# stephanieleroux/sitrack

Measured on AMD Instinct MI355X. Metric: particle-steps/s, higher is better.
Workload: dtype f64

## Files before the change

include/sitrk.h:

```cpp
#ifndef SITRK_H
#define SITRK_H

#include <stdint.h>

#ifdef __cplusplus
extern "C" {
#endif

#define SITRK_VERSION 100

#define SITRK_OK        0
#define SITRK_EINVAL  (-1)
#define SITRK_EINDEX  (-2)
#define SITRK_EHIP    (-3)
#define SITRK_ENOMEM  (-4)

#define SITRK_F32 0
#define SITRK_F64 1

#define SITRK_FILL (-9999.0)

typedef struct sitrk_ctx sitrk_t;

int         sitrk_version(void);
// ... 1 lines not shown
int         sitrk_destroy(sitrk_t *h);
const char *sitrk_last_error(sitrk_t *h);
int         sitrk_sync(sitrk_t *h);
int         sitrk_set_stream(sitrk_t *h, void *hip_stream);

int sitrk_set_grid(sitrk_t *h, int Nj, int Ni,
                   const double *Yf, const double *Xf,
                   const double *Yu, const double *Xu,
                   const double *Yv, const double *Xv,
                   const int8_t *tmask);

int sitrk_set_params(sitrk_t *h, double rdt, int uv_strategy, double rmin_conc);

int sitrk_set_substeps(sitrk_t *h, int nsub);

int sitrk_set_tuning(sitrk_t *h, const char *knob, int value);

int   sitrk_alloc_records(sitrk_t *h, int nslots, int dtype);
int   sitrk_push_record(sitrk_t *h, int slot, const void *u, const void *v, const void *sic);
int   sitrk_stage_acquire(sitrk_t *h, int nrows, void **u, void **v, void **sic);
int   sitrk_stage_submit(sitrk_t *h, int slot, int j0, int j1);
int   sitrk_stage_release(sitrk_t *h);
int   sitrk_push_record_dev(sitrk_t *h, int slot, const void *slab_dev);
void *sitrk_record_ptr(sitrk_t *h, int slot);
int   sitrk_commit_record(sitrk_t *h, int slot);

int sitrk_buoy_rows(sitrk_t *h, int32_t *jmin, int32_t *jmax);
int sitrk_push_record_rows(sitrk_t *h, int slot, int j0, int j1, const void *u_rows, const void *v_rows, const void *sic_rows);
int sitrk_commit_record_rows(sitrk_t *h, int slot, int j0, int j1);

int sitrk_buoy_box(sitrk_t *h, int32_t *jmin, int32_t *jmax, int32_t *imin, int32_t *imax);
int sitrk_push_record_box(sitrk_t *h, int slot, int j0, int j1, int i0, int i1, const void *u_box, const void *v_box, const void *sic_box,
                          int64_t ld);
int sitrk_buoy_box_begin(sitrk_t *h);
int sitrk_buoy_box_end(sitrk_t *h, int32_t *jmin, int32_t *jmax, int32_t *imin, int32_t *imax, int32_t *age);
int sitrk_stage_acquire_box(sitrk_t *h, int nrows, int ncols, void **u, void **v, void **sic);
int sitrk_stage_submit_box(sitrk_t *h, int slot, int j0, int j1, int i0, int i1);
int sitrk_commit_record_box(sitrk_t *h, int slot, int j0, int j1, int i0, int i1);
int sitrk_commit_records_box(sitrk_t *h, int slot0, int nrec, int j0, int j1, int i0, int i1);
int sitrk_commit_records_box_async(sitrk_t *h, int slot0, int nrec, int j0, int j1, int i0, int i1);

int sitrk_set_buoys(sitrk_t *h, int64_t nP, const double *yx, const int32_t *jiT,
                    const int32_t *rec_first, const int32_t *rec_last);

int sitrk_restore_state(sitrk_t *h, const int8_t *alive, const int32_t *kill_rec);

int sitrk_sort_buoys(sitrk_t *h);
int sitrk_set_resort(sitrk_t *h, int resort_every);

int sitrk_step(sitrk_t *h, int slot, int jrec);

int sitrk_run(sitrk_t *h, int slot0, int jrec0, int nsteps);
int sitrk_launch_stats(sitrk_t *h, int reset, int64_t *fused_launches, int64_t *fused_records, int64_t *step_launches);

int sitrk_fetch(sitrk_t *h, double *yx, int32_t *jiT, int8_t *alive, int32_t *kill_rec);

int sitrk_fetch_record(sitrk_t *h, int jrec, double *yx_rec, int8_t *mask, double *latlon);

int sitrk_find_cells(sitrk_t *h, int64_t n, const double *yx, const int32_t *jiT_guess,
                     int32_t *jiT_out, int8_t *found);

int sitrk_seed_init(sitrk_t *h, int64_t nP, const double *latlon, const double *yx,
                    const double *latT, const double *lonT, const double *resolkm,
                    const double *sic, int32_t *jiT_out, int8_t *keep, int8_t *why);

int sitrk_nearest_point(sitrk_t *h, int64_t nP, const double *latlon, const double *latT, const double *lonT,
                        const double *resolkm, double rd_found_km, int max_itr, int32_t *ji, double *dmin);

int sitrk_nemo_seed(sitrk_t *h, int Nj, int Ni, int khss, const int8_t *tmask, const int8_t *rmask,
                    const double *latT, const double *lonT, const double *sic, const double *latF, const double *lonF,
                    double lat0, double lon0, int64_t capacity, double *latlon, double *yx, int64_t *nT, int64_t *nF);

int sitrk_subsample_cloud(sitrk_t *h, int64_t n, const double *yx, double rd_km, int8_t *keep, int64_t *nkeep, int32_t *launches);

int sitrk_cancel_too_close(sitrk_t *h, int64_t n, const double *lat, const double *lon, const int8_t *valid, const int32_t *nrec_all,
                           const int32_t *nrec_before, double rd_km, int8_t *keep, int64_t *nkeep, int64_t *nclose);

int sitrk_nearest_buoy(sitrk_t *h, int64_t n, const double *lat, const double *lon, const int8_t *valid, double rd_km, int32_t *nn,
                       double *dmin);

int sitrk_eval_inside(sitrk_t *h, int64_t n, const double *pts, const double *quads, int8_t *inside);
int sitrk_eval_euler(sitrk_t *h, int64_t n, const double *r, const double *vel, double rdt, double *out);
int sitrk_eval_haversine(sitrk_t *h, int64_t n, const double *plat, const double *plon, const double *xlat,
                         const double *xlon, double *dist);
int sitrk_eval_intersect(sitrk_t *h, int64_t n, const double *segs, int8_t *intersect, int8_t *ccw_abc);
int sitrk_eval_crossing(sitrk_t *h, int64_t n, const double *P1, const double *P2, const int32_t *jiT, int32_t *jiT_new,
                        int32_t *codes);
int sitrk_survive_mask(sitrk_t *h, const double *sic, int8_t *mask);

int sitrk_cart2geo(sitrk_t *h, int64_t n, const double *yx, double lat0, double lon0, double *latlon);
int sitrk_geo2cart(sitrk_t *h, int64_t n, const double *latlon, double lat0, double lon0, double *yx);

int sitrk_timer_start(sitrk_t *h);
int sitrk_timer_stop(sitrk_t *h, float *ms);
int sitrk_count_alive(sitrk_t *h, int64_t *nalive);

#ifdef __cplusplus
}
#endif
#endif
```

sitrack_amd/_lib.py:

```python
import ctypes as C
import os
import subprocess

import numpy as np

_HERE = os.path.dirname(os.path.abspath(__file__))
SO_PATH = os.environ.get("SITRK_LIB_PATH") or os.path.join(_HERE, "libsitrk.so")
CSRC = os.path.join(_HERE, "csrc")

SITRK_F32, SITRK_F64 = 0, 1
FillValue = -9999.0

_vp = C.c_void_p
_i64 = C.c_int64
_int = C.c_int
_dbl = C.c_double

_SIGNATURES = {
    "sitrk_version": (_int, []),
    "sitrk_create": (_int, [C.POINTER(_vp), _int]),
    "sitrk_destroy": (_int, [_vp]),
    "sitrk_last_error": (C.c_char_p, [_vp]),
    "sitrk_sync": (_int, [_vp]),
    "sitrk_set_stream": (_int, [_vp, _vp]),
    "sitrk_set_grid": (_int, [_vp, _int, _int] + [_vp] * 7),
    "sitrk_set_params": (_int, [_vp, _dbl, _int, _dbl]),
    "sitrk_set_substeps": (_int, [_vp, _int]),
    "sitrk_set_tuning": (_int, [_vp, C.c_char_p, _int]),
    "sitrk_alloc_records": (_int, [_vp, _int, _int]),
    "sitrk_push_record": (_int, [_vp, _int, _vp, _vp, _vp]),
    "sitrk_push_record_dev": (_int, [_vp, _int, _vp]),
    "sitrk_stage_acquire": (_int, [_vp, _int, C.POINTER(_vp), C.POINTER(_vp), C.POINTER(_vp)]),
    "sitrk_stage_submit": (_int, [_vp, _int, _int, _int]),
    "sitrk_stage_release": (_int, [_vp]),
    "sitrk_launch_stats": (_int, [_vp, _int, C.POINTER(_i64), C.POINTER(_i64), C.POINTER(_i64)]),
    "sitrk_buoy_rows": (_int, [_vp, C.POINTER(C.c_int32), C.POINTER(C.c_int32)]),
    "sitrk_push_record_rows": (_int, [_vp, _int, _int, _int, _vp, _vp, _vp]),
    "sitrk_commit_record_rows": (_int, [_vp, _int, _int, _int]),
    "sitrk_buoy_box": (_int, [_vp] + [C.POINTER(C.c_int32)] * 4),
    "sitrk_push_record_box": (_int, [_vp, _int, _int, _int, _int, _int, _vp, _vp, _vp, _i64]),
    "sitrk_buoy_box_begin": (_int, [_vp]),
    "sitrk_buoy_box_end": (_int, [_vp] + [C.POINTER(C.c_int32)] * 5),
    "sitrk_stage_acquire_box": (_int, [_vp, _int, _int, C.POINTER(_vp), C.POINTER(_vp), C.POINTER(_vp)]),
    "sitrk_stage_submit_box": (_int, [_vp, _int, _int, _int, _int, _int]),
    "sitrk_commit_record_box": (_int, [_vp, _int, _int, _int, _int, _int]),
    "sitrk_commit_records_box": (_int, [_vp, _int, _int, _int, _int, _int, _int]),
    "sitrk_commit_records_box_async": (_int, [_vp, _int, _int, _int, _int, _int, _int]),
    "sitrk_record_ptr": (_vp, [_vp, _int]),
    "sitrk_commit_record": (_int, [_vp, _int]),
    "sitrk_set_buoys": (_int, [_vp, _i64, _vp, _vp, _vp, _vp]),
    "sitrk_restore_state": (_int, [_vp, _vp, _vp]),
    "sitrk_sort_buoys": (_int, [_vp]),
    "sitrk_set_resort": (_int, [_vp, _int]),
    "sitrk_step": (_int, [_vp, _int, _int]),
    "sitrk_run": (_int, [_vp, _int, _int, _int]),
    "sitrk_fetch": (_int, [_vp, _vp, _vp, _vp, _vp]),
    "sitrk_fetch_record": (_int, [_vp, _int, _vp, _vp, _vp]),
    "sitrk_count_alive": (_int, [_vp, C.POINTER(_i64)]),
    "sitrk_find_cells": (_int, [_vp, _i64, _vp, _vp, _vp, _vp]),
    "sitrk_seed_init": (_int, [_vp, _i64] + [_vp] * 9),
    "sitrk_nemo_seed": (_int, [_vp, _int, _int, _int] + [_vp] * 7 + [_dbl, _dbl, _i64, _vp, _vp, C.POINTER(_i64), C.POINTER(_i64)]),
    "sitrk_subsample_cloud": (_int, [_vp, _i64, _vp, _dbl, _vp, C.POINTER(_i64), C.POINTER(C.c_int32)]),
    "sitrk_cancel_too_close": (_int, [_vp, _i64, _vp, _vp, _vp, _vp, _vp, _dbl, _vp, C.POINTER(_i64), C.POINTER(_i64)]),
    "sitrk_nearest_buoy": (_int, [_vp, _i64, _vp, _vp, _vp, _dbl, _vp, _vp]),
    "sitrk_nearest_point": (_int, [_vp, _i64, _vp, _vp, _vp, _vp, _dbl, _int, _vp, _vp]),
    "sitrk_eval_haversine": (_int, [_vp, _i64, _vp, _vp, _vp, _vp, _vp]),
    "sitrk_eval_inside": (_int, [_vp, _i64, _vp, _vp, _vp]),
    "sitrk_eval_euler": (_int, [_vp, _i64, _vp, _vp, _dbl, _vp]),
    "sitrk_eval_intersect": (_int, [_vp, _i64, _vp, _vp, _vp]),
    "sitrk_eval_crossing": (_int, [_vp, _i64, _vp, _vp, _vp, _vp, _vp]),
    "sitrk_survive_mask": (_int, [_vp, _vp, _vp]),
    "sitrk_cart2geo": (_int, [_vp, _i64, _vp, _dbl, _dbl, _vp]),
    "sitrk_geo2cart": (_int, [_vp, _i64, _vp, _dbl, _dbl, _vp]),
    "sitrk_timer_start": (_int, [_vp]),
    "sitrk_timer_stop": (_int, [_vp, C.POINTER(C.c_float)]),
}


class SitrkError(RuntimeError):
    pass


def build(force=False, verbose=False):
    cmd = ["make", "-C", CSRC] + (["-B"] if force else [])
    r = subprocess.run(cmd, capture_output=True, text=True)
    if verbose or r.returncode:
        print(r.stdout + r.stderr)
    if r.returncode:
# ... 131 lines not shown
            raise ValueError("records must be float32 or float64")
        self._chk(self._L.sitrk_alloc_records(self._h, int(nslots), SITRK_F64 if dt == np.float64 else SITRK_F32))
        self.nslots = int(nslots)
        self.field_dtype = dt

    def push_record(self, slot, u, v, sic):
        shp = (self.Nj, self.Ni)
        u = as_c(u, self.field_dtype, shp, "u")
        v = as_c(v, self.field_dtype, shp, "v")
        sic = as_c(sic, self.field_dtype, shp, "sic")
        self._chk(self._L.sitrk_push_record(self._h, int(slot), _ptr(u), _ptr(v), _ptr(sic)))

    def stage(self, nrows=None, ncols=None):
        nrows = self.Nj if nrows is None else int(nrows)
        ncols = self.Ni if ncols is None else int(ncols)
        pu, pv, ps = _vp(), _vp(), _vp()
        if ncols == self.Ni:
            self._chk(self._L.sitrk_stage_acquire(self._h, nrows, C.byref(pu), C.byref(pv), C.byref(ps)))
        else:
            self._chk(self._L.sitrk_stage_acquire_box(self._h, nrows, ncols, C.byref(pu), C.byref(pv), C.byref(ps)))
        nb = nrows * ncols * self.field_dtype.itemsize

        def view(p):
            return np.frombuffer((C.c_char * nb).from_address(p.value), dtype=self.field_dtype).reshape(nrows, ncols)
        self._staged_rows, self._staged_cols = nrows, ncols
        return view(pu), view(pv), view(ps)

    def stage_release(self):
        self._chk(self._L.sitrk_stage_release(self._h))

    def stage_fill(self, slot, j0, nrows, fill, i0=0, ncols=None):
        bufs = self.stage(nrows, ncols)
        try:
            fill(*bufs)
        except BaseException:
            self.stage_release()
            raise
        finally:
            del bufs
        self.submit(slot, j0, i0)

    def submit(self, slot, j0=0, i0=0):
        j1, i1 = int(j0) + int(self._staged_rows), int(i0) + int(self._staged_cols)
        if int(i0) == 0 and i1 == self.Ni:
            self._chk(self._L.sitrk_stage_submit(self._h, int(slot), int(j0), j1))
        else:
            self._chk(self._L.sitrk_stage_submit_box(self._h, int(slot), int(j0), j1, int(i0), i1))

    def launch_stats(self, reset=False):
        a, b, c = _i64(0), _i64(0), _i64(0)
        self._chk(self._L.sitrk_launch_stats(self._h, int(bool(reset)), C.byref(a), C.byref(b), C.byref(c)))
        return {"fused_launches": a.value, "fused_records": b.value, "step_launches": c.value}

    def buoy_rows(self):
        a, b = C.c_int32(0), C.c_int32(0)
        self._chk(self._L.sitrk_buoy_rows(self._h, C.byref(a), C.byref(b)))
        return a.value, b.value

    def band(self, age=0):
        jmin, jmax = self.buoy_rows()
        if jmin > jmax:
            return 0, 0
        d = reach(age, self.nsub)
        return max(0, jmin - 2 - d), min(self.Nj, jmax + 3 + d)

    def buoy_box(self):
        v = [C.c_int32(0) for _ in range(4)]
        self._chk(self._L.sitrk_buoy_box(self._h, *[C.byref(x) for x in v]))
        return tuple(x.value for x in v)

    def box(self, age=0, align=4):
        jmin, jmax, imin, imax = self.buoy_box()
        return self.box_of(jmin, jmax, imin, imax, age, align)

    def box_of(self, jmin, jmax, imin, imax, age=0, align=4):
        if jmin > jmax:
            return 0, 0, 0, 0
        d = reach(age, getattr(self, "nsub", 1))
        i0, i1 = max(0, imin - 2 - d), min(self.Ni, imax + 3 + d)
        i0 -= i0 % align
        i1 = min(self.Ni, -(-i1 // align) * align)
        return max(0, jmin - 2 - d), min(self.Nj, jmax + 3 + d), i0, i1

    def push_record_box(self, slot, j0, j1, i0, i1, u_box, v_box, sic_box):
        shp = (j1 - j0, i1 - i0)
        es = self.field_dtype.itemsize
        arrs = [np.asarray(x) for x in (u_box, v_box, sic_box)]
        for x, n in zip(arrs, ("u box", "v box", "sic box")):
            if tuple(x.shape) != shp:
                raise ValueError("%s: expected shape %s, got %s" % (n, shp, tuple(x.shape)))
        pitched = all(x.dtype == self.field_dtype and x.ndim == 2 and x.strides[1] == es and x.strides[0] % es == 0
                      and x.strides[0] >= shp[1] * es for x in arrs) and len({x.strides[0] for x in arrs}) == 1
        if pitched and shp[0] > 0 and shp[1] > 0:
            ld = arrs[0].strides[0] // es
        else:
            arrs = [as_c(x, self.field_dtype, shp) for x in arrs]
            ld = shp[1]
        self._chk(self._L.sitrk_push_record_box(self._h, int(slot), int(j0), int(j1), int(i0), int(i1), *[_ptr(x) for x in arrs], int(ld)))

    def buoy_box_begin(self):
        self._chk(self._L.sitrk_buoy_box_begin(self._h))

    def buoy_box_end(self):
        v = [C.c_int32(0) for _ in range(5)]
        self._chk(self._L.sitrk_buoy_box_end(self._h, *[C.byref(x) for x in v]))
        return tuple(x.value for x in v)
# ... 259 lines not shown
```

sitrack_amd/csrc/sitrk.hip:

```cpp
#include <hip/hip_runtime.h>

#include <algorithm>
#include <cmath>
#include <cstdarg>
#include <cstdio>
#include <cstring>
#include <new>
#include <thread>
#include <vector>

#include "../../include/sitrk.h"
#include "sitrk_internal.h"
#include "sitrk_kernels.h"
#include "sitrk_locate.h"
#include "sitrk_seed.h"

using namespace sitrk;

#define SITRK_API extern "C" __attribute__((visibility("default")))

static thread_local char g_create_err[512] = {0};

static int fail(sitrk_ctx *h, int code, const char *fmt, ...)
{
// ... 36 lines not shown
    dev_free(h->scratch);
    h->scratch = nullptr;
    h->scratch_bytes = 0;
    HIPCHK(hipMalloc(&h->scratch, bytes));
    h->scratch_bytes = bytes;
    return SITRK_OK;
}

static void free_buoys(sitrk_ctx *h)
{
    for (int b = 0; b < 2; b++) {
        dev_free(h->st[b].pos); dev_free(h->st[b].cell); dev_free(h->st[b].kill_rec);
        dev_free(h->st[b].win); dev_free(h->st[b].perm);
        h->st[b] = BuoyState();
        dev_free(h->keys[b]); dev_free(h->vals[b]);
        h->keys[b] = nullptr; h->vals[b] = nullptr;
    }
    dev_free(h->sort_tmp);
    h->sort_tmp = nullptr; h->sort_tmp_bytes = 0;
    h->nP = 0;
}

static void free_records(sitrk_ctx *h);

SITRK_API int sitrk_version(void) { return SITRK_VERSION; }

SITRK_API const char *sitrk_last_error(sitrk_t *h) { return h ? h->err : g_create_err; }

SITRK_API int sitrk_create(sitrk_t **out, int device)
{
    sitrk_ctx *h = nullptr;
    if (!out) return fail(h, SITRK_EINVAL, "sitrk_create: null output pointer");
    *out = nullptr;
    int ndev = 0;
    hipError_t e = hipGetDeviceCount(&ndev);
    if (e != hipSuccess || ndev <= 0)
        return fail(h, SITRK_EHIP, "sitrk_create: no HIP device (%s); libsitrk has no CPU path",
                    e == hipSuccess ? "device count 0" : hipGetErrorString(e));
    if (device < 0 || device >= ndev) return fail(h, SITRK_EINVAL, "sitrk_create: device %d out of range [0,%d)", device, ndev);
    e = hipSetDevice(device);
    if (e != hipSuccess) return fail(h, SITRK_EHIP, "hipSetDevice(%d) -> %s", device, hipGetErrorString(e));
    sitrk_ctx *c = new (std::nothrow) sitrk_ctx();
    if (!c) return fail(h, SITRK_ENOMEM, "sitrk_create: out of host memory");
    c->device = device;
    for (int k = 0; k < 4096; k++) c->slot_used_seq[k] = -1;
    e = hipStreamCreateWithFlags(&c->own_stream, hipStreamNonBlocking);
    if (e == hipSuccess) e = hipStreamCreateWithFlags(&c->copy_stream, hipStreamNonBlocking);
    if (e == hipSuccess) e = hipStreamCreateWithFlags(&c->sv_stream, hipStreamNonBlocking);
    if (e == hipSuccess) e = hipEventCreate(&c->ev0);
    if (e == hipSuccess) e = hipEventCreate(&c->ev1);
    for (int b = 0; b < sitrk_ctx::kStage && e == hipSuccess; b++) e = hipEventCreateWithFlags(&c->stage_done[b], hipEventDisableTiming);
    for (int k = 0; k < sitrk_ctx::kLaunchRing && e == hipSuccess; k++) e = hipEventCreateWithFlags(&c->launch_ev[k], hipEventDisableTiming);
    if (e == hipSuccess) e = hipEventCreateWithFlags(&c->box_ev, hipEventDisableTiming);
    if (e == hipSuccess) e = hipHostMalloc((void **)&c->box_host, 4 * sizeof(int), hipHostMallocDefault);
    if (e == hipSuccess) e = hipMalloc((void **)&c->counter, 4 * sizeof(unsigned long long));
    if (e != hipSuccess) {
        int rc = fail(h, SITRK_EHIP, "sitrk_create: %s", hipGetErrorString(e));
        (void)sitrk_destroy(c);
        return rc;
    }
    c->stream = c->own_stream;
    *out = c;
    return SITRK_OK;
}

SITRK_API int sitrk_destroy(sitrk_t *h)
{
    if (!h) return SITRK_OK;
    (void)hipSetDevice(h->device);
    if (h->copy_stream) (void)hipStreamSynchronize(h->copy_stream);
    if (h->sv_stream) (void)hipStreamSynchronize(h->sv_stream);
    if (h->stream) (void)hipStreamSynchronize(h->stream);
    free_buoys(h);
    free_records(h);
    dev_free(h->geo); dev_free(h->geoF); dev_free(h->orient); dev_free(h->tmask); dev_free(h->scratch); dev_free(h->counter);
    if (h->box_ev) (void)hipEventDestroy(h->box_ev);
    if (h->box_host) (void)hipHostFree(h->box_host);
    if (h->ev0) (void)hipEventDestroy(h->ev0);
    if (h->ev1) (void)hipEventDestroy(h->ev1);
    for (int b = 0; b < sitrk_ctx::kStage; b++) if (h->stage_done[b]) (void)hipEventDestroy(h->stage_done[b]);
    for (int k = 0; k < sitrk_ctx::kLaunchRing; k++) if (h->launch_ev[k]) (void)hipEventDestroy(h->launch_ev[k]);
    for (int k = 0; k < 4096; k++) if (h->slot_ready[k]) (void)hipEventDestroy(h->slot_ready[k]);
    for (int k = 0; k < 4096; k++) if (h->slot_sv[k]) (void)hipEventDestroy(h->slot_sv[k]);
    if (h->sv_stream) (void)hipStreamDestroy(h->sv_stream);
    if (h->copy_stream) (void)hipStreamDestroy(h->copy_stream);
    if (h->own_stream) (void)hipStreamDestroy(h->own_stream);
    delete h;
    return SITRK_OK;
}

SITRK_API int sitrk_sync(sitrk_t *h)
{
    NEED(h, "null handle");
    HIPCHK(hipStreamSynchronize(h->copy_stream));
    HIPCHK(hipStreamSynchronize(h->sv_stream));
    HIPCHK(hipStreamSynchronize(h->stream));
    return SITRK_OK;
}

SITRK_API int sitrk_set_stream(sitrk_t *h, void *hip_stream)
{
    NEED(h, "null handle");
    HIPCHK(hipStreamSynchronize(h->stream));
    h->stream = hip_stream ? (hipStream_t)hip_stream : h->own_stream;
    return SITRK_OK;
}

SITRK_API int sitrk_set_grid(sitrk_t *h, int Nj, int Ni, const double *Yf, const double *Xf, const double *Yu,
                             const double *Xu, const double *Yv, const double *Xv, const int8_t *tmask)
{
    NEED(h, "null handle");
    NEED(Yf && Xf && Yu && Xu && Yv && Xv && tmask, "sitrk_set_grid: null array");
    if (Nj < 4 || Nj > 32767 || Ni < 4 || Ni > 65535)
        return fail(h, SITRK_EINVAL, "sitrk_set_grid: grid %dx%d outside 4..32767 x 4..65535", Nj, Ni);
    if ((int64_t)Nj * Ni > ((int64_t)1 << 29))
        return fail(h, SITRK_EINVAL, "sitrk_set_grid: grid %dx%d has more than 2^29 cells", Nj, Ni);
    HIPCHK(hipSetDevice(h->device));
    HIPCHK(hipStreamSynchronize(h->copy_stream));
    HIPCHK(hipStreamSynchronize(h->sv_stream));
    HIPCHK(hipStreamSynchronize(h->stream));
    dev_free(h->geo); dev_free(h->geoF); dev_free(h->orient); dev_free(h->tmask);
    h->geo = nullptr; h->geoF = nullptr; h->orient = nullptr; h->tmask = nullptr;
    free_records(h);
    free_buoys(h);
    const size_t n = (size_t)Nj * Ni;
    HIPCHK(dev_alloc(&h->geo, n));
    HIPCHK(dev_alloc(&h->geoF, n));
    HIPCHK(dev_alloc(&h->orient, n));
    HIPCHK(dev_alloc(&h->tmask, n));
// ... 16 lines not shown
    }
    h->eps_mg = 0x1p-48 * mg;
    HIPCHK(hipStreamSynchronize(h->stream));
    h->Nj = Nj; h->Ni = Ni;
    return SITRK_OK;
}

SITRK_API int sitrk_set_params(sitrk_t *h, double rdt, int uv_strategy, double rmin_conc)
{
    NEED(h, "null handle");
    NEED(uv_strategy >= 0 && uv_strategy <= 2,
         "sitrk_set_params: uv_strategy must be 0 (cell mean), 1 (nearest U/V point) or 2 (linear interpolation, not in the reference)");
    NEED(rdt > 0.0, "sitrk_set_params: rdt must be > 0");
    if (rmin_conc != h->rmin_conc) memset(h->slot_dirty, 1, sizeof(h->slot_dirty));
    h->rdt = rdt; h->uv_strategy = uv_strategy; h->rmin_conc = rmin_conc;
    return SITRK_OK;
}

SITRK_API int sitrk_set_substeps(sitrk_t *h, int nsub)
{
    NEED(h, "null handle");
    NEED(nsub >= 1 && nsub <= 1024, "sitrk_set_substeps: nsub must be in 1..1024");
    h->nsub = nsub;
    return SITRK_OK;
}

SITRK_API int sitrk_set_tuning(sitrk_t *h, const char *knob, int value)
{
    NEED(h, "null handle");
    NEED(knob, "sitrk_set_tuning: null knob");
    int bit = 0;
    if (!strcmp(knob, "xcd_remap")) bit = TUNE_XCD_REMAP;
    else if (!strcmp(knob, "nt_state")) bit = TUNE_NT_STATE;
    else if (!strcmp(knob, "survive_tile")) bit = TUNE_SURVIVE_TILE;
    else if (!strcmp(knob, "step_block")) {
        if (value != 256 && value != 512 && value != 1024) return fail(h, SITRK_EINVAL, "sitrk_set_tuning: step_block must be 256, 512 or 1024");
        h->step_block = value;
        return SITRK_OK;
    }
    else if (!strcmp(knob, "fuse")) {
        if (value < 1 || value > kMaxFuse) return fail(h, SITRK_EINVAL, "sitrk_set_tuning: fuse must be 1..%d", kMaxFuse);
        h->fuse = value;
        return SITRK_OK;
    }
    else if (!strcmp(knob, "sort_tile")) {
        const int tj = value >> 8, ti = value & 255;
        if (value != 0 && (tj < 1 || ti < 1)) return fail(h, SITRK_EINVAL, "sitrk_set_tuning: sort_tile = tile_j*256 + tile_i");
        h->tile_j = tj; h->tile_i = ti;
        return SITRK_OK;
    }
    else if (!strcmp(knob, "patch_kb")) {
        if (value < 0 || value > 63) return fail(h, SITRK_EINVAL, "sitrk_set_tuning: patch_kb must be 0..63");
        h->patch_kb = value;
        return SITRK_OK;
    }
    else if (!strcmp(knob, "xcd_group")) {
        if (value < 0 || value > 4096) return fail(h, SITRK_EINVAL, "sitrk_set_tuning: xcd_group must be 0..4096");
        h->xcd_group = value;
        return SITRK_OK;
    }
    else if (!strcmp(knob, "async_survive")) {
        h->async_survive = value != 0;
        return SITRK_OK;
    }
    else if (!strcmp(knob, "fill_threads")) {
        if (value < 1 || value > 16) return fail(h, SITRK_EINVAL, "sitrk_set_tuning: fill_threads must be 1..16");
        h->fill_threads = value;
        return SITRK_OK;
    }
    else if (!strcmp(knob, "patch_margin")) {
        if (value < 0 || value > 64) return fail(h, SITRK_EINVAL, "sitrk_set_tuning: patch_margin must be 0..64");
        h->patch_margin = value;
        return SITRK_OK;
    }
    else if (!strcmp(knob, "subsample_block")) {
        if (value < 256 || value > 256 * kSubMaxPpt || (value & (value - 1)))
            return fail(h, SITRK_EINVAL, "sitrk_set_tuning: subsample_block must be a power of two in 256..%d", 256 * kSubMaxPpt);
        h->subsample_block = value;
        return SITRK_OK;
    }
    else if (!strcmp(knob, "locate_bruteforce")) bit = TUNE_LOCATE_BRUTEFORCE;
    else return fail(h, SITRK_EINVAL, "sitrk_set_tuning: unknown knob '%s'", knob);
    h->tune = value ? (h->tune | bit) : (h->tune & ~bit);
    return SITRK_OK;
}

static inline size_t elem_size(int dtype) { return dtype == SITRK_F64 ? 8 : 4; }

static void free_records(sitrk_ctx *h)
{
    dev_free(h->slabs); dev_free(h->kill9);
    h->slabs = nullptr; h->kill9 = nullptr; h->nslots = 0;
    for (int b = 0; b < sitrk_ctx::kStage; b++) {
        if (h->stage[b]) (void)hipHostFree(h->stage[b]);
        h->stage[b] = nullptr;
    }
    h->stage_bytes = 0; h->stage_rows = -1; h->stage_cols = 0; h->stage_next = 0;
    memset(h->slot_pending, 0, sizeof(h->slot_pending));
    memset(h->slot_sv_pending, 0, sizeof(h->slot_sv_pending));
    memset(h->slot_dirty, 1, sizeof(h->slot_dirty));
    for (int k = 0; k < 4096; k++) {
        h->slot_used_seq[k] = -1;
        h->slot_row_lo[k] = h->slot_row_hi[k] = 0;
        h->slot_col_lo[k] = h->slot_col_hi[k] = 0;
    }
}
// ... 643 lines not shown
    HIPCHK(sort_pairs_u32(nullptr, &need, h->keys[0], h->keys[1], h->vals[0], h->vals[1], (size_t)nP, end_bit, h->stream));
    if (need > h->sort_tmp_bytes) {
        HIPCHK(hipStreamSynchronize(h->stream));
        dev_free(h->sort_tmp);
        h->sort_tmp = nullptr; h->sort_tmp_bytes = 0;
        HIPCHK(hipMalloc(&h->sort_tmp, need));
        h->sort_tmp_bytes = need;
    }
    size_t tb = h->sort_tmp_bytes;
    HIPCHK(sort_pairs_u32(h->sort_tmp, &tb, h->keys[0], h->keys[1], h->vals[0], h->vals[1], (size_t)nP, end_bit, h->stream));
    hipLaunchKernelGGL(permute_state_kernel, dim3(nblocks(nP)), dim3(kBlock), 0, h->stream, nP, h->vals[1], h->keys[1], dead_key, h->Ni, h->tile_j, h->tile_i,
                       in, out, h->windowed);
    HIPCHK(hipGetLastError());
    h->cur ^= 1;
    h->sorted_once = true;
    return SITRK_OK;
}

static inline bool window_test_needed(const sitrk_ctx *h, int jrec0, int n)
{
    return h->windowed && !(jrec0 >= h->win_first_max && (int64_t)jrec0 + n - 1 <= h->win_last_min);
}

template <typename FT, int BLOCK>
static void launch_step_b(sitrk_ctx *h, const StepArgs &a)
{
    const bool windowed = window_test_needed(h, a.jrec, 1);
    dim3 grid(nblocks(a.nP, BLOCK)), block(BLOCK);
    if (h->uv_strategy == 1) {
        if (windowed) hipLaunchKernelGGL((advect_step_kernel<FT, 1, true, BLOCK>), grid, block, 0, h->stream, a);
        else hipLaunchKernelGGL((advect_step_kernel<FT, 1, false, BLOCK>), grid, block, 0, h->stream, a);
    } else if (h->uv_strategy == 2) {
        if (windowed) hipLaunchKernelGGL((advect_step_kernel<FT, 2, true, BLOCK>), grid, block, 0, h->stream, a);
        else hipLaunchKernelGGL((advect_step_kernel<FT, 2, false, BLOCK>), grid, block, 0, h->stream, a);
    } else {
        if (windowed) hipLaunchKernelGGL((advect_step_kernel<FT, 0, true, BLOCK>), grid, block, 0, h->stream, a);
        else hipLaunchKernelGGL((advect_step_kernel<FT, 0, false, BLOCK>), grid, block, 0, h->stream, a);
    }
}

template <typename FT>
static void launch_step(sitrk_ctx *h, const StepArgs &a)
{
    if (h->step_block == 1024) launch_step_b<FT, 1024>(h, a);
    else if (h->step_block == 512) launch_step_b<FT, 512>(h, a);
    else launch_step_b<FT, 256>(h, a);
}

static inline bool fused_ok(const sitrk_ctx *h)
{
    return !h->rim_buoys && (uint64_t)h->Nj * h->Ni * sizeof(CellGeo) < ((uint64_t)1 << 32);
}

static int launch_records(sitrk_ctx *h, int slot_first, int jrec0, int m);

SITRK_API int sitrk_step(sitrk_t *h, int slot, int jrec)
{
    NEED(h, "null handle");
    NEED(h->st[0].pos, "sitrk_step: call sitrk_set_buoys first");
    NEED(h->slabs, "sitrk_step: call sitrk_alloc_records first");
    NEED(slot >= 0 && slot < h->nslots, "sitrk_step: slot out of range");
    if (h->nP == 0) return SITRK_OK;
    int rc = check_band(h, slot, 0);
    if (rc) return rc;
    if (h->resort_every > 0 && h->steps_since_sort >= h->resort_every) {
        rc = sitrk_sort_buoys(h);
        if (rc) return rc;
    }
    if (h->slot_dirty[slot]) {
        rc = derive_mask(h, slot);
        if (rc) return rc;
    }
    rc = slot_wait_upload(h, slot);
    if (rc) return rc;
    rc = slot_wait_sv(h, slot);
    if (rc) return rc;
    if (h->nsub > 1 && fused_ok(h)) return launch_records(h, slot, jrec, 1);
    const size_t n = (size_t)h->Nj * h->Ni, es = elem_size(h->dtype);
    const char *slab = slab_of(h, slot);
    BuoyState &s = h->st[h->cur];
    StepArgs a;
    a.nP = h->nP; a.tune = h->tune; a.Nj = h->Nj; a.Ni = h->Ni; a.jrec = jrec;
    a.rdt = h->rdt; a.rmin_conc = h->rmin_conc; a.eps_mg = h->eps_mg;
    a.geo = h->geo; a.orient = h->orient; a.kill = h->kill9 + (size_t)slot * n;
    a.u = slab; a.v = slab + n * es;
    a.pos = s.pos; a.cell = s.cell; a.kill_rec = s.kill_rec; a.win = s.win;
    if (h->nsub > 1) a.rdt = h->rdt / h->nsub;
    for (int sub = 0; sub < h->nsub; sub++) {
        if (h->dtype == SITRK_F64) launch_step<double>(h, a);
        else launch_step<float>(h, a);
        HIPCHK(hipGetLastError());
    }
    rc = launch_mark(h, &slot, 1);
    if (rc) return rc;
    h->steps_since_sort++;
    h->n_step_launches += h->nsub;
    if (h->band_age >= 0) h->band_age++;
    if (h->box_pending) h->box_pending_age++;
    return SITRK_OK;
}

static int f32_class_for(double rdt)
{
    const double ar = std::fabs(rdt);
    return (ar >= 0x1p-700 && ar <= 0x1p700) ? kClassFiniteNonzeroF32 : 0;
}

template <typename FT>
static void launch_run(sitrk_ctx *h, const RunArgs &ra)
{
    dim3 grid(nblocks(ra.s.nP, kRunBlock)), block(kRunBlock);
    const size_t lds = kRunLdsFixed + (size_t)ra.patch_cells * sizeof(pt);
    const bool windowed = window_test_needed(h, ra.s.jrec, ra.nrec);
    if (h->uv_strategy == 1) {
        if (windowed) hipLaunchKernelGGL((advect_run_kernel<FT, 1, true>), grid, block, lds, h->stream, ra);
        else hipLaunchKernelGGL((advect_run_kernel<FT, 1, false>), grid, block, lds, h->stream, ra);
    } else if (h->uv_strategy == 2) {
        if (windowed) hipLaunchKernelGGL((advect_run_kernel<FT, 2, true>), grid, block, lds, h->stream, ra);
        else hipLaunchKernelGGL((advect_run_kernel<FT, 2, false>), grid, block, lds, h->stream, ra);
    } else {
        if (windowed) hipLaunchKernelGGL((advect_run_kernel<FT, 0, true>), grid, block, lds, h->stream, ra);
        else hipLaunchKernelGGL((advect_run_kernel<FT, 0, false>), grid, block, lds, h->stream, ra);
    }
}

template <typename FT>
static void launch_substep(sitrk_ctx *h, const RunArgs &ra, int nsub)
{
    dim3 grid(nblocks(ra.s.nP, kRunBlock)), block(kRunBlock);
    const size_t lds = kRunLdsFixed + (size_t)ra.patch_cells * sizeof(pt);
    const bool windowed = window_test_needed(h, ra.s.jrec, ra.nrec);
    if (h->uv_strategy == 1) {
        if (windowed) hipLaunchKernelGGL((advect_substep_kernel<FT, 1, true>), grid, block, lds, h->stream, ra, nsub);
        else hipLaunchKernelGGL((advect_substep_kernel<FT, 1, false>), grid, block, lds, h->stream, ra, nsub);
    } else if (h->uv_strategy == 2) {
        if (windowed) hipLaunchKernelGGL((advect_substep_kernel<FT, 2, true>), grid, block, lds, h->stream, ra, nsub);
        else hipLaunchKernelGGL((advect_substep_kernel<FT, 2, false>), grid, block, lds, h->stream, ra, nsub);
    } else {
        if (windowed) hipLaunchKernelGGL((advect_substep_kernel<FT, 0, true>), grid, block, lds, h->stream, ra, nsub);
        else hipLaunchKernelGGL((advect_substep_kernel<FT, 0, false>), grid, block, lds, h->stream, ra, nsub);
    }
}

static int launch_records(sitrk_ctx *h, int slot_first, int jrec0, int m)
{
    BuoyState &s = h->st[h->cur];
    const size_t n = (size_t)h->Nj * h->Ni, es = elem_size(h->dtype);
    const double dt = h->nsub > 1 ? h->rdt / h->nsub : h->rdt;
    RunArgs ra;
    ra.s.nP = h->nP; ra.s.tune = h->tune; ra.s.Nj = h->Nj; ra.s.Ni = h->Ni; ra.s.jrec = jrec0;
    ra.s.rdt = dt; ra.s.rmin_conc = h->rmin_conc; ra.s.eps_mg = h->eps_mg; ra.s.geo = h->geo; ra.s.orient = h->orient; ra.s.kill = nullptr; ra.s.u = ra.s.v = nullptr;
    ra.s.pos = s.pos; ra.s.cell = s.cell; ra.s.kill_rec = s.kill_rec; ra.s.win = s.win;
    ra.nrec = m;
    make_cross_tab(h->Ni, ra.tab, ra.dji);
    ra.geoF = h->geoF;
    ra.patch_cells = (int)((size_t)h->patch_kb * 1024 / sizeof(pt));
    ra.patch_margin = h->patch_margin;
    ra.xcd_group = h->xcd_group;
    ra.f32_class = f32_class_for(dt);
    int used[kMaxFuse];
    for (int r = 0; r < m; r++) {
        const int slot = (slot_first + r) % h->nslots;
        used[r] = slot;
        int rc = check_band(h, slot, r);
        if (rc) return rc;
        if (h->slot_dirty[slot]) {
            rc = derive_mask(h, slot);
            if (rc) return rc;
        }
        rc = slot_wait_upload(h, slot);
        if (rc) return rc;
        rc = slot_wait_sv(h, slot);
        if (rc) return rc;
        const char *slab = slab_of(h, slot);
        ra.u[r] = slab; ra.v[r] = slab + n * es; ra.kill9[r] = h->kill9 + (size_t)slot * n;
    }
    if (h->nsub > 1) {
        if (h->dtype == SITRK_F64) launch_substep<double>(h, ra, h->nsub);
        else launch_substep<float>(h, ra, h->nsub);
    } else {
        if (h->dtype == SITRK_F64) launch_run<double>(h, ra);
        else launch_run<float>(h, ra);
    }
    HIPCHK(hipGetLastError());
    int rc = launch_mark(h, used, m);
    if (rc) return rc;
    h->steps_since_sort += m;
    h->n_fused_launches++;
    h->n_fused_records += m;
    if (h->band_age >= 0) h->band_age += m;
    if (h->box_pending) h->box_pending_age += m;
    return SITRK_OK;
}

SITRK_API int sitrk_run(sitrk_t *h, int slot0, int jrec0, int nsteps)
{
    NEED(h, "null handle");
    NEED(nsteps >= 0, "sitrk_run: nsteps must be >= 0");
    NEED(h->nslots > 0, "sitrk_run: call sitrk_alloc_records first");
    NEED(slot0 >= 0 && slot0 < h->nslots, "sitrk_run: slot0 out of range");
    NEED(h->st[0].pos, "sitrk_run: call sitrk_set_buoys first");
    if (h->nP == 0) return SITRK_OK;
    int fuse = std::max(1, std::min(std::min(h->fuse, kMaxFuse), h->nslots));
    if (!fused_ok(h)) fuse = 1;
    int k = 0;
    while (k < nsteps) {
        if (h->resort_every > 0 && h->steps_since_sort >= h->resort_every) {
            int rc = sitrk_sort_buoys(h);
            if (rc) return rc;
        }
        int m = std::min(fuse, nsteps - k);
        if (h->resort_every > 0) m = std::min(m, h->resort_every - h->steps_since_sort);
        if (m <= 1) {
            int rc = sitrk_step(h, (slot0 + k) % h->nslots, jrec0 + k);
            if (rc) return rc;
            k += 1;
            continue;
        }
        int rc = launch_records(h, (slot0 + k) % h->nslots, jrec0 + k, m);
        if (rc) return rc;
        k += m;
    }
    return SITRK_OK;
}

SITRK_API int sitrk_launch_stats(sitrk_t *h, int reset, int64_t *fused_launches, int64_t *fused_records, int64_t *step_launches)
{
    NEED(h, "null handle");
    if (fused_launches) *fused_launches = h->n_fused_launches;
    if (fused_records) *fused_records = h->n_fused_records;
    if (step_launches) *step_launches = h->n_step_launches;
    if (reset) h->n_fused_launches = h->n_fused_records = h->n_step_launches = 0;
    return SITRK_OK;
}

SITRK_API int sitrk_fetch(sitrk_t *h, double *yx, int32_t *jiT, int8_t *alive, int32_t *kill_rec)
{
    NEED(h, "null handle");
    NEED(h->st[0].pos, "sitrk_fetch: call sitrk_set_buoys first");
    const int64_t nP = h->nP;
    if (nP == 0) return SITRK_OK;
    HIPCHK(hipSetDevice(h->device));
    const size_t b_yx = align256((size_t)nP * sizeof(pt)), b_ji = align256((size_t)nP * 8), b_al = align256((size_t)nP),
                 b_kr = align256((size_t)nP * 4);
    int rc = ensure_scratch(h, b_yx + b_ji + b_al + b_kr);
    if (rc) return rc;
    char *s = (char *)h->scratch;
    pt *d_yx = yx ? (pt *)s : nullptr;
    int32_t *d_ji = jiT ? (int32_t *)(s + b_yx) : nullptr;
    int8_t *d_al = alive ? (int8_t *)(s + b_yx + b_ji) : nullptr;
    int32_t *d_kr = kill_rec ? (int32_t *)(s + b_yx + b_ji + b_al) : nullptr;
    hipLaunchKernelGGL(fetch_state_kernel, dim3(nblocks(nP)), dim3(kBlock), 0, h->stream, nP, h->st[h->cur], d_yx, d_ji, d_al, d_kr);
    HIPCHK(hipGetLastError());
    if (yx) HIPCHK(hipMemcpyAsync(yx, d_yx, (size_t)nP * sizeof(pt), hipMemcpyDeviceToHost, h->stream));
    if (jiT) HIPCHK(hipMemcpyAsync(jiT, d_ji, (size_t)nP * 8, hipMemcpyDeviceToHost, h->stream));
    if (alive) HIPCHK(hipMemcpyAsync(alive, d_al, (size_t)nP, hipMemcpyDeviceToHost, h->stream));
    if (kill_rec) HIPCHK(hipMemcpyAsync(kill_rec, d_kr, (size_t)nP * 4, hipMemcpyDeviceToHost, h->stream));
    HIPCHK(hipStreamSynchronize(h->stream));
    return SITRK_OK;
}

static ProjParams make_proj(double lat0, double lon0)
{
    ProjParams pp;
    const double f = 1.0 / 298.257223563;
    pp.a = 6378137.0;
    pp.e = std::sqrt(2.0 * f - f * f);
    pp.lon0 = lon0;
    const double phits = std::fabs(lat0) * (M_PI / 180.0);
    if (std::fabs(phits - M_PI_2) < 1e-10) {
        pp.akm1 = 2.0 / std::sqrt(std::pow(1 + pp.e, 1 + pp.e) * std::pow(1 - pp.e, 1 - pp.e));
    } else {
        double t = std::sin(phits);
        double es = pp.e * t;
        double tsfn = std::tan(0.5 * (M_PI_2 - phits)) / std::pow((1.0 - es) / (1.0 + es), 0.5 * pp.e);
        pp.akm1 = std::cos(phits) / tsfn;
        pp.akm1 /= std::sqrt(1.0 - es * es);
    }
    return pp;
}

SITRK_API int sitrk_fetch_record(sitrk_t *h, int jrec, double *yx_rec, int8_t *mask, double *latlon)
{
    NEED(h, "null handle");
    NEED(h->st[0].pos, "sitrk_fetch_record: call sitrk_set_buoys first");
// ... 743 lines not shown
```

sitrack_amd/csrc/sitrk_internal.h:

```cpp
#pragma once
#include <hip/hip_runtime.h>
#include <stdint.h>
#include <stddef.h>

#include "sitrk_geom.h"

namespace sitrk {

hipError_t sort_pairs_u32(void *tmp, size_t *tmp_bytes, const uint32_t *kin, uint32_t *kout,
                          const int32_t *vin, int32_t *vout, size_t n, unsigned end_bit, hipStream_t s);

struct SubGrid {
    double ymin = 0.0, xmin = 0.0, inv_h = 0.0;
    int ny = 1, nx = 1;
};
constexpr int kSubMaxPpt = 16;
struct SubResolveArgs {
    SubGrid g;
    int64_t n = 0;
    double r2 = 0.0;
    int ppt = 4;
    const pt *yx = nullptr;
    const int32_t *perm = nullptr;
    const int32_t *cstart = nullptr, *cend = nullptr;
// ... 24 lines not shown
                              const int32_t *perm, V3 *uv_s, ll *ll_s, int32_t *cstart, int32_t *cend, hipStream_t s);
hipError_t overlap_nearest(const OvGrid &g, int64_t n, double rd_km, double cut2, const uint32_t *key_sorted, const int32_t *perm,
                           const V3 *uv_s, const ll *ll_s, const int32_t *cstart, const int32_t *cend, int32_t *nn, double *dmin,
                           hipStream_t s);
hipError_t overlap_compact(void *tmp, size_t *tmp_bytes, int64_t n, const int32_t *nn, int32_t *flag, int32_t *pos, int32_t *cidx,
                           int32_t *cnn, hipStream_t s);

struct BuoyState {
    pt      *pos      = nullptr;
    int32_t *cell     = nullptr;
    int32_t *kill_rec = nullptr;
    int2    *win      = nullptr;
    int32_t *perm     = nullptr;
};

}

struct sitrk_ctx {
    int device = 0;
    char err[512] = {0};

    hipStream_t own_stream = nullptr;
    hipStream_t stream = nullptr;
    hipStream_t copy_stream = nullptr;
    hipStream_t sv_stream = nullptr;
    hipEvent_t ev0 = nullptr, ev1 = nullptr;

    static constexpr int kStage = 2;
    void *stage[kStage] = {nullptr, nullptr};
    size_t stage_bytes = 0;
    hipEvent_t stage_done[kStage] = {nullptr, nullptr};
    int stage_next = 0;
    int stage_rows = -1;
    int stage_cols = 0;

    int Nj = 0, Ni = 0;
    sitrk::CellGeo *geo = nullptr;
    sitrk::pt *geoF = nullptr;
    int8_t *orient = nullptr;
    int8_t *tmask = nullptr;

    double rdt = 3600.0;
    int nsub = 1;
    int uv_strategy = 1;
    double rmin_conc = 0.1;
    double eps_mg = 0.0;
    int tune = sitrk::TUNE_NT_STATE;
    int step_block = 512;
    int fuse = 32;
    int tile_j = 8, tile_i = 16;
    int patch_kb = 16;
    int xcd_group = 16;
    int patch_margin = 8;
    int subsample_block = 1024;
    int fill_threads = 8;

    int nslots = 0, dtype = 0;
    size_t slab_bytes = 0;
    void *slabs = nullptr;
    uint8_t *kill9 = nullptr;
    unsigned char slot_dirty[4096] = {0};
    unsigned char slot_pending[4096] = {0};
    hipEvent_t slot_ready[4096] = {nullptr};
    hipEvent_t slot_sv[4096] = {nullptr};
    unsigned char slot_sv_pending[4096] = {0};
    int async_survive = 0;
    long long slot_used_seq[4096];
    static constexpr int kLaunchRing = 64;
    hipEvent_t launch_ev[kLaunchRing] = {nullptr};
    long long launch_seq = 0;
    int slot_row_lo[4096] = {0}, slot_row_hi[4096] = {0};
    int slot_col_lo[4096] = {0}, slot_col_hi[4096] = {0};
    int band_jmin = 0, band_jmax = -1, band_age = -1;
    int band_imin = 0, band_imax = -1;
    int *box_host = nullptr;
    hipEvent_t box_ev = nullptr;
    bool box_pending = false;
    int box_pending_age = 0;
    long long n_fused_launches = 0, n_fused_records = 0, n_step_launches = 0;

    int64_t nP = 0;
    bool windowed = false;
    int32_t win_first_max = 0, win_last_min = 0;
    bool rim_buoys = false;
    sitrk::BuoyState st[2];
    int cur = 0;
    uint32_t *keys[2] = {nullptr, nullptr};
    int32_t *vals[2] = {nullptr, nullptr};
    void *sort_tmp = nullptr;
    size_t sort_tmp_bytes = 0;
    int resort_every = 512;
    int steps_since_sort = 0;
    bool sorted_once = false;

    void *scratch = nullptr;
    size_t scratch_bytes = 0;
    unsigned long long *counter = nullptr;
};
```

Measured before the change: 163.7 billion.

## Split buoy set into two stream lanes with staggered fused launches

Partitions the particles into two halves and launches the fused advection kernels for each half on separate streams (main and sv_stream), staggering the second lane by half a fuse so the tail of one launch overlaps the start of the next. Slot preparation and bookkeeping are hoisted into a per-segment prepare step with a fork/join event pair. The aim is to hide the kernel-boundary tail drain and launch gaps. In exchange it adds cross-stream scheduling complexity and reuses sv_stream, and it only engages when the second half has enough workgroups (lane_min_wg).

```diff
diff --git a/include/sitrk.h b/include/sitrk.h
--- a/include/sitrk.h
+++ b/include/sitrk.h
@@ -77,6 +77,7 @@
 
 int sitrk_run(sitrk_t *h, int slot0, int jrec0, int nsteps);
 int sitrk_launch_stats(sitrk_t *h, int reset, int64_t *fused_launches, int64_t *fused_records, int64_t *step_launches);
+int sitrk_lane_stats(sitrk_t *h, int reset, int64_t *lane_segments, int64_t *lane_launches);
 
 int sitrk_fetch(sitrk_t *h, double *yx, int32_t *jiT, int8_t *alive, int32_t *kill_rec);
 
diff --git a/sitrack_amd/_lib.py b/sitrack_amd/_lib.py
--- a/sitrack_amd/_lib.py
+++ b/sitrack_amd/_lib.py
@@ -34,6 +34,7 @@
     "sitrk_stage_submit": (_int, [_vp, _int, _int, _int]),
     "sitrk_stage_release": (_int, [_vp]),
     "sitrk_launch_stats": (_int, [_vp, _int, C.POINTER(_i64), C.POINTER(_i64), C.POINTER(_i64)]),
+    "sitrk_lane_stats": (_int, [_vp, _int, C.POINTER(_i64), C.POINTER(_i64)]),
     "sitrk_buoy_rows": (_int, [_vp, C.POINTER(C.c_int32), C.POINTER(C.c_int32)]),
     "sitrk_push_record_rows": (_int, [_vp, _int, _int, _int, _vp, _vp, _vp]),
     "sitrk_commit_record_rows": (_int, [_vp, _int, _int, _int]),
@@ -271,6 +272,11 @@
         self._chk(self._L.sitrk_launch_stats(self._h, int(bool(reset)), C.byref(a), C.byref(b), C.byref(c)))
         return {"fused_launches": a.value, "fused_records": b.value, "step_launches": c.value}
 
+    def lane_stats(self, reset=False):
+        a, b = _i64(0), _i64(0)
+        self._chk(self._L.sitrk_lane_stats(self._h, int(bool(reset)), C.byref(a), C.byref(b)))
+        return {"lane_segments": a.value, "lane_launches": b.value}
+
     def buoy_rows(self):
         a, b = C.c_int32(0), C.c_int32(0)
         self._chk(self._L.sitrk_buoy_rows(self._h, C.byref(a), C.byref(b)))
diff --git a/sitrack_amd/csrc/sitrk.hip b/sitrack_amd/csrc/sitrk.hip
--- a/sitrack_amd/csrc/sitrk.hip
+++ b/sitrack_amd/csrc/sitrk.hip
@@ -112,6 +112,8 @@
     for (int b = 0; b < sitrk_ctx::kStage && e == hipSuccess; b++) e = hipEventCreateWithFlags(&c->stage_done[b], hipEventDisableTiming);
     for (int k = 0; k < sitrk_ctx::kLaunchRing && e == hipSuccess; k++) e = hipEventCreateWithFlags(&c->launch_ev[k], hipEventDisableTiming);
     if (e == hipSuccess) e = hipEventCreateWithFlags(&c->box_ev, hipEventDisableTiming);
+    if (e == hipSuccess) e = hipEventCreateWithFlags(&c->lane_fork, hipEventDisableTiming);
+    if (e == hipSuccess) e = hipEventCreateWithFlags(&c->lane_join, hipEventDisableTiming);
     if (e == hipSuccess) e = hipHostMalloc((void **)&c->box_host, 4 * sizeof(int), hipHostMallocDefault);
     if (e == hipSuccess) e = hipMalloc((void **)&c->counter, 4 * sizeof(unsigned long long));
     if (e != hipSuccess) {
@@ -135,6 +137,8 @@
     free_records(h);
     dev_free(h->geo); dev_free(h->geoF); dev_free(h->orient); dev_free(h->tmask); dev_free(h->scratch); dev_free(h->counter);
     if (h->box_ev) (void)hipEventDestroy(h->box_ev);
+    if (h->lane_fork) (void)hipEventDestroy(h->lane_fork);
+    if (h->lane_join) (void)hipEventDestroy(h->lane_join);
     if (h->box_host) (void)hipHostFree(h->box_host);
     if (h->ev0) (void)hipEventDestroy(h->ev0);
     if (h->ev1) (void)hipEventDestroy(h->ev1);
@@ -257,6 +261,16 @@
     else if (!strcmp(knob, "patch_kb")) {
         if (value < 0 || value > 63) return fail(h, SITRK_EINVAL, "sitrk_set_tuning: patch_kb must be 0..63");
         h->patch_kb = value;
+        return SITRK_OK;
+    }
+    else if (!strcmp(knob, "lanes")) {
+        if (value < 1 || value > 2) return fail(h, SITRK_EINVAL, "sitrk_set_tuning: lanes must be 1 or 2");
+        h->lanes = value;
+        return SITRK_OK;
+    }
+    else if (!strcmp(knob, "lane_min_wg")) {
+        if (value < 1) return fail(h, SITRK_EINVAL, "sitrk_set_tuning: lane_min_wg must be >= 1");
+        h->lane_min_wg = value;
         return SITRK_OK;
     }
     else if (!strcmp(knob, "xcd_group")) {
@@ -1006,7 +1020,7 @@
     return !h->rim_buoys && (uint64_t)h->Nj * h->Ni * sizeof(CellGeo) < ((uint64_t)1 << 32);
 }
 
-static int launch_records(sitrk_ctx *h, int slot_first, int jrec0, int m);
+static int launch_records(sitrk_ctx *h, int slot_first, int jrec0, int m, int64_t off = 0, int64_t cnt = -1, hipStream_t lane = nullptr);
 
 SITRK_API int sitrk_step(sitrk_t *h, int slot, int jrec)
 {
@@ -1061,50 +1075,52 @@
 }
 
 template <typename FT>
-static void launch_run(sitrk_ctx *h, const RunArgs &ra)
+static void launch_run(sitrk_ctx *h, const RunArgs &ra, hipStream_t stream)
 {
     dim3 grid(nblocks(ra.s.nP, kRunBlock)), block(kRunBlock);
     const size_t lds = kRunLdsFixed + (size_t)ra.patch_cells * sizeof(pt);
     const bool windowed = window_test_needed(h, ra.s.jrec, ra.nrec);
     if (h->uv_strategy == 1) {
-        if (windowed) hipLaunchKernelGGL((advect_run_kernel<FT, 1, true>), grid, block, lds, h->stream, ra);
-        else hipLaunchKernelGGL((advect_run_kernel<FT, 1, false>), grid, block, lds, h->stream, ra);
+        if (windowed) hipLaunchKernelGGL((advect_run_kernel<FT, 1, true>), grid, block, lds, stream, ra);
+        else hipLaunchKernelGGL((advect_run_kernel<FT, 1, false>), grid, block, lds, stream, ra);
     } else if (h->uv_strategy == 2) {
-        if (windowed) hipLaunchKernelGGL((advect_run_kernel<FT, 2, true>), grid, block, lds, h->stream, ra);
-        else hipLaunchKernelGGL((advect_run_kernel<FT, 2, false>), grid, block, lds, h->stream, ra);
+        if (windowed) hipLaunchKernelGGL((advect_run_kernel<FT, 2, true>), grid, block, lds, stream, ra);
+        else hipLaunchKernelGGL((advect_run_kernel<FT, 2, false>), grid, block, lds, stream, ra);
     } else {
-        if (windowed) hipLaunchKernelGGL((advect_run_kernel<FT, 0, true>), grid, block, lds, h->stream, ra);
-        else hipLaunchKernelGGL((advect_run_kernel<FT, 0, false>), grid, block, lds, h->stream, ra);
+        if (windowed) hipLaunchKernelGGL((advect_run_kernel<FT, 0, true>), grid, block, lds, stream, ra);
+        else hipLaunchKernelGGL((advect_run_kernel<FT, 0, false>), grid, block, lds, stream, ra);
     }
 }
 
 template <typename FT>
-static void launch_substep(sitrk_ctx *h, const RunArgs &ra, int nsub)
+static void launch_substep(sitrk_ctx *h, const RunArgs &ra, int nsub, hipStream_t stream)
 {
     dim3 grid(nblocks(ra.s.nP, kRunBlock)), block(kRunBlock);
     const size_t lds = kRunLdsFixed + (size_t)ra.patch_cells * sizeof(pt);
     const bool windowed = window_test_needed(h, ra.s.jrec, ra.nrec);
     if (h->uv_strategy == 1) {
-        if (windowed) hipLaunchKernelGGL((advect_substep_kernel<FT, 1, true>), grid, block, lds, h->stream, ra, nsub);
-        else hipLaunchKernelGGL((advect_substep_kernel<FT, 1, false>), grid, block, lds, h->stream, ra, nsub);
+        if (windowed) hipLaunchKernelGGL((advect_substep_kernel<FT, 1, true>), grid, block, lds, stream, ra, nsub);
+        else hipLaunchKernelGGL((advect_substep_kernel<FT, 1, false>), grid, block, lds, stream, ra, nsub);
     } else if (h->uv_strategy == 2) {
-        if (windowed) hipLaunchKernelGGL((advect_substep_kernel<FT, 2, true>), grid, block, lds, h->stream, ra, nsub);
-        else hipLaunchKernelGGL((advect_substep_kernel<FT, 2, false>), grid, block, lds, h->stream, ra, nsub);
+        if (windowed) hipLaunchKernelGGL((advect_substep_kernel<FT, 2, true>), grid, block, lds, stream, ra, nsub);
+        else hipLaunchKernelGGL((advect_substep_kernel<FT, 2, false>), grid, block, lds, stream, ra, nsub);
     } else {
-        if (windowed) hipLaunchKernelGGL((advect_substep_kernel<FT, 0, true>), grid, block, lds, h->stream, ra, nsub);
-        else hipLaunchKernelGGL((advect_substep_kernel<FT, 0, false>), grid, block, lds, h->stream, ra, nsub);
-    }
-}
-
-static int launch_records(sitrk_ctx *h, int slot_first, int jrec0, int m)
+        if (windowed) hipLaunchKernelGGL((advect_substep_kernel<FT, 0, true>), grid, block, lds, stream, ra, nsub);
+        else hipLaunchKernelGGL((advect_substep_kernel<FT, 0, false>), grid, block, lds, stream, ra, nsub);
+    }
+}
+
+static int launch_records(sitrk_ctx *h, int slot_first, int jrec0, int m, int64_t off, int64_t cnt, hipStream_t lane)
 {
     BuoyState &s = h->st[h->cur];
+    const hipStream_t stream = lane ? lane : h->stream;
+    if (cnt < 0) cnt = h->nP - off;
     const size_t n = (size_t)h->Nj * h->Ni, es = elem_size(h->dtype);
     const double dt = h->nsub > 1 ? h->rdt / h->nsub : h->rdt;
     RunArgs ra;
-    ra.s.nP = h->nP; ra.s.tune = h->tune; ra.s.Nj = h->Nj; ra.s.Ni = h->Ni; ra.s.jrec = jrec0;
+    ra.s.nP = cnt; ra.s.tune = h->tune; ra.s.Nj = h->Nj; ra.s.Ni = h->Ni; ra.s.jrec = jrec0;
     ra.s.rdt = dt; ra.s.rmin_conc = h->rmin_conc; ra.s.eps_mg = h->eps_mg; ra.s.geo = h->geo; ra.s.orient = h->orient; ra.s.kill = nullptr; ra.s.u = ra.s.v = nullptr;
-    ra.s.pos = s.pos; ra.s.cell = s.cell; ra.s.kill_rec = s.kill_rec; ra.s.win = s.win;
+    ra.s.pos = s.pos + off; ra.s.cell = s.cell + off; ra.s.kill_rec = s.kill_rec + off; ra.s.win = s.win ? s.win + off : nullptr;
     ra.nrec = m;
     make_cross_tab(h->Ni, ra.tab, ra.dji);
     ra.geoF = h->geoF;
@@ -1116,27 +1132,30 @@
     for (int r = 0; r < m; r++) {
         const int slot = (slot_first + r) % h->nslots;
         used[r] = slot;
-        int rc = check_band(h, slot, r);
-        if (rc) return rc;
-        if (h->slot_dirty[slot]) {
-            rc = derive_mask(h, slot);
+        if (!lane) {
+            int rc = check_band(h, slot, r);
+            if (rc) return rc;
+            if (h->slot_dirty[slot]) {
+                rc = derive_mask(h, slot);
+                if (rc) return rc;
+            }
+            rc = slot_wait_upload(h, slot);
+            if (rc) return rc;
+            rc = slot_wait_sv(h, slot);
             if (rc) return rc;
         }
-        rc = slot_wait_upload(h, slot);
-        if (rc) return rc;
-        rc = slot_wait_sv(h, slot);
-        if (rc) return rc;
         const char *slab = slab_of(h, slot);
         ra.u[r] = slab; ra.v[r] = slab + n * es; ra.kill9[r] = h->kill9 + (size_t)slot * n;
     }
     if (h->nsub > 1) {
-        if (h->dtype == SITRK_F64) launch_substep<double>(h, ra, h->nsub);
-        else launch_substep<float>(h, ra, h->nsub);
+        if (h->dtype == SITRK_F64) launch_substep<double>(h, ra, h->nsub, stream);
+        else launch_substep<float>(h, ra, h->nsub, stream);
     } else {
-        if (h->dtype == SITRK_F64) launch_run<double>(h, ra);
-        else launch_run<float>(h, ra);
-    }
-    HIPCHK(hipGetLastError());
+        if (h->dtype == SITRK_F64) launch_run<double>(h, ra, stream);
+        else launch_run<float>(h, ra, stream);
+    }
+    HIPCHK(hipGetLastError());
+    if (lane) return SITRK_OK;
     int rc = launch_mark(h, used, m);
     if (rc) return rc;
     h->steps_since_sort += m;
@@ -1144,6 +1163,75 @@
     h->n_fused_records += m;
     if (h->band_age >= 0) h->band_age += m;
     if (h->box_pending) h->box_pending_age += m;
+    return SITRK_OK;
+}
+
+
+static int64_t lane_cut(const sitrk_ctx *h)
+{
+    if (h->lanes < 2) return 0;
+    const int64_t unit = (int64_t)kRunBlock * 8 * std::max(1, h->xcd_group);
+    const int64_t cut = ((h->nP + unit - 1) / unit + 1) / 2 * unit;
+    if (cut >= h->nP) return 0;
+    return (h->nP - cut + kRunBlock - 1) / kRunBlock >= h->lane_min_wg ? cut : 0;
+}
+
+static int lanes_prepare(sitrk_ctx *h, int slot_first, int seg, bool *ok)
+{
+    *ok = false;
+    for (int q = 0; q < seg; q++)
+        if (check_band(h, (slot_first + q) % h->nslots, q)) return SITRK_OK;
+    for (int q = 0; q < std::min(seg, h->nslots); q++) {
+        const int slot = (slot_first + q) % h->nslots;
+        int rc = SITRK_OK;
+        if (h->slot_dirty[slot]) rc = derive_mask(h, slot);
+        if (!rc) rc = slot_wait_upload(h, slot);
+        if (!rc) rc = slot_wait_sv(h, slot);
+        if (rc) return rc;
+    }
+    for (int k = 0; k < h->nslots; k++)
+        if (h->slot_sv_pending[k]) return SITRK_OK;
+    *ok = true;
+    return SITRK_OK;
+}
+
+static int run_lanes(sitrk_ctx *h, int slot_first, int jrec0, int seg, int fuse, int64_t cut)
+{
+    const hipStream_t l1 = h->sv_stream;
+    HIPCHK(hipEventRecord(h->lane_fork, h->stream));
+    HIPCHK(hipStreamWaitEvent(l1, h->lane_fork, 0));
+    int rc = SITRK_OK;
+    int a = 0, b = 0;
+    while (rc == SITRK_OK && (a < seg || b < seg)) {
+        if (a < seg && (a <= b || b >= seg)) {
+            const int m = std::min(fuse, seg - a);
+            rc = launch_records(h, (slot_first + a) % h->nslots, jrec0 + a, m, 0, cut, h->stream);
+            a += m;
+            h->n_lane_launches++;
+        } else {
+            const int m = std::min(b == 0 ? fuse / 2 : fuse, seg - b);
+            rc = launch_records(h, (slot_first + b) % h->nslots, jrec0 + b, m, cut, h->nP - cut, l1);
+            b += m;
+            h->n_lane_launches++;
+        }
+    }
+    hipError_t e = hipEventRecord(h->lane_join, l1);
+    if (e == hipSuccess) e = hipStreamWaitEvent(h->stream, h->lane_join, 0);
+    if (rc) return rc;
+    HIPCHK(e);
+    const long long seq = ++h->launch_seq;
+    HIPCHK(hipEventRecord(h->launch_ev[seq % sitrk_ctx::kLaunchRing], h->stream));
+    for (int q = 0; q < std::min(seg, h->nslots); q++) h->slot_used_seq[(slot_first + q) % h->nslots] = seq;
+    for (int q = 0; q < seg;) {
+        const int m = std::min(fuse, seg - q);
+        if (m <= 1 && h->nsub == 1) h->n_step_launches++;
+        else { h->n_fused_launches++; h->n_fused_records += m; }
+        q += m;
+    }
+    h->n_lane_segments++;
+    h->steps_since_sort += seg;
+    if (h->band_age >= 0) h->band_age += seg;
+    if (h->box_pending) h->box_pending_age += seg;
     return SITRK_OK;
 }
 
@@ -1157,11 +1245,27 @@
     if (h->nP == 0) return SITRK_OK;
     int fuse = std::max(1, std::min(std::min(h->fuse, kMaxFuse), h->nslots));
     if (!fused_ok(h)) fuse = 1;
+    const int64_t cut = fuse >= 2 ? lane_cut(h) : 0;
     int k = 0;
     while (k < nsteps) {
         if (h->resort_every > 0 && h->steps_since_sort >= h->resort_every) {
             int rc = sitrk_sort_buoys(h);
             if (rc) return rc;
+        }
+        if (cut > 0) {
+            int seg = nsteps - k;
+            if (h->resort_every > 0) seg = std::min(seg, h->resort_every - h->steps_since_sort);
+            bool ok = false;
+            if (seg >= 2 * fuse + fuse / 2) {
+                int rc = lanes_prepare(h, (slot0 + k) % h->nslots, seg, &ok);
+                if (rc) return rc;
+            }
+            if (ok) {
+                int rc = run_lanes(h, (slot0 + k) % h->nslots, jrec0 + k, seg, fuse, cut);
+                if (rc) return rc;
+                k += seg;
+                continue;
+            }
         }
         int m = std::min(fuse, nsteps - k);
         if (h->resort_every > 0) m = std::min(m, h->resort_every - h->steps_since_sort);
@@ -1185,6 +1289,15 @@
     if (fused_records) *fused_records = h->n_fused_records;
     if (step_launches) *step_launches = h->n_step_launches;
     if (reset) h->n_fused_launches = h->n_fused_records = h->n_step_launches = 0;
+    return SITRK_OK;
+}
+
+SITRK_API int sitrk_lane_stats(sitrk_t *h, int reset, int64_t *lane_segments, int64_t *lane_launches)
+{
+    NEED(h, "null handle");
+    if (lane_segments) *lane_segments = h->n_lane_segments;
+    if (lane_launches) *lane_launches = h->n_lane_launches;
+    if (reset) h->n_lane_segments = h->n_lane_launches = 0;
     return SITRK_OK;
 }
 
diff --git a/sitrack_amd/csrc/sitrk_internal.h b/sitrack_amd/csrc/sitrk_internal.h
--- a/sitrack_amd/csrc/sitrk_internal.h
+++ b/sitrack_amd/csrc/sitrk_internal.h
@@ -100,6 +100,9 @@
     int patch_kb = 16;
     int xcd_group = 16;
     int patch_margin = 8;
+    int lanes = 2;
+    int lane_min_wg = 7168;
+    hipEvent_t lane_fork = nullptr, lane_join = nullptr;
     int subsample_block = 1024;
     int fill_threads = 8;
 
@@ -126,6 +129,7 @@
     bool box_pending = false;
     int box_pending_age = 0;
     long long n_fused_launches = 0, n_fused_records = 0, n_step_launches = 0;
+    long long n_lane_segments = 0, n_lane_launches = 0;
 
     int64_t nP = 0;
     bool windowed = false;
```

Result: faster. 167.0 billion (median of 6 runs) (+2.0%).
